# lukifer23/Matrix0

Measured on AMD Instinct MI355X. Metric: self-play games/sec at 800 sims/move, ResNet-24 53M; 1/2/4/8 MI355X, higher is better.
Workload: dtype f16

## Files before the change

matrix0_amd/csrc/attn_block.hip:

```cpp
#include "attn_math.h"
#include "conv_epilogue.h"

typedef float float4v __attribute__((ext_vector_type(4)));

namespace {
constexpr int AB_PIECE = 12288;
constexpr int AB_PIECES_PER_GROUP = 7;
constexpr int AB_GROUPS = 10;
constexpr int AB_X = 0;
constexpr int AB_QK = 81920;
constexpr int AB_VT = AB_QK + 16384;
constexpr int AB_VROW = 68;
constexpr int AB_RING = AB_VT + 4 * 16 * AB_VROW * 2;
constexpr int AB_PAR = AB_RING + 4 * AB_PIECE;
constexpr int AB_LDS = AB_PAR + 4 * 320 * 4;

struct AbLane {
    int tid, lane, w;
    int l15, lq, r31, half;
    int wm, wn;
    size_t b0;
    uint32_t xa[2];
    int wq0, wq1, wpo;
    uint32_t ring_a, of_a;
    const char* wsrc;
    char* ring_w;
    int au, aboard, ahl, aqt, aq;
};
struct AbRegs {
    float4v oc[20];
    float4v qa[2][3];
    half8 fs[2][5];
    half8 of;
    half8 bias8[4];
    half2v visp[16];
};
}

__device__ __forceinline__ void ab_load64(half8& b0, half8& b1, half8& b2, half8& b3, const half8* p) {
    asm volatile("global_load_dwordx4 %0, %4, off\n\tglobal_load_dwordx4 %1, %4, off offset:16\n\t"
                 "global_load_dwordx4 %2, %4, off offset:32\n\tglobal_load_dwordx4 %3, %4, off offset:48"
                 : "=&v"(b0), "=&v"(b1), "=&v"(b2), "=&v"(b3) : "v"(p) : "memory");
}
template <int OFF>
__device__ __forceinline__ void ab_lds16(half8& d, uint32_t addr) {
    asm volatile("ds_read_b128 %0, %1 offset:%2" : "=v"(d) : "v"(addr), "n"(OFF) : "memory");
}
template <int N>
__device__ __forceinline__ void ab_lds_arrived(half8& f0, half8& f1, half8& f2, half8& f3, half8& f4, half8& f5) {
    static_assert(N == 0 || N == 5, "");
    if constexpr (N == 0) asm volatile("s_waitcnt lgkmcnt(0)" : "+v"(f0), "+v"(f1), "+v"(f2), "+v"(f3), "+v"(f4), "+v"(f5) :: "memory");
    else asm volatile("s_waitcnt lgkmcnt(5)" : "+v"(f0), "+v"(f1), "+v"(f2), "+v"(f3), "+v"(f4), "+v"(f5) :: "memory");
}
template <int CTRL>
__device__ __forceinline__ float ab_dpp(float v) {
    return __builtin_bit_cast(float, __builtin_amdgcn_update_dpp(0, __builtin_bit_cast(int, v), CTRL, 0xF, 0xF, true));
}
__device__ __forceinline__ float ab_row_sum(float v) {
    v += ab_dpp<0xB1>(v);
    v += ab_dpp<0x4E>(v);
    v += ab_dpp<0x141>(v);
    v += ab_dpp<0x140>(v);
    return v;
}

#define AB_WAIT(n) asm volatile("s_waitcnt vmcnt(" #n ")" ::: "memory")
#define AB_LGKM0() asm volatile("s_waitcnt lgkmcnt(0)" ::: "memory")

__device__ __forceinline__ char* ab_smem() {
    extern __shared__ __attribute__((aligned(16))) char smem[];
    return smem;
}

__device__ __forceinline__ AbLane ab_lane(const AttnBlockArgs& a) {
    AbLane L;
    L.tid = threadIdx.x; L.lane = L.tid & 63;
    L.w = __builtin_amdgcn_readfirstlane(L.tid >> 6);
    L.l15 = L.lane & 15; L.lq = L.lane >> 4; L.r31 = L.lane & 31; L.half = L.lane >> 5;
    L.wm = L.w >> 1; L.wn = L.w & 1;
    L.b0 = (size_t)blockIdx.x * 2;
    const int l15 = L.l15, lq = L.lq, w = L.w;
    const int xrow0 = 32 * L.wm + l15;
    const int xsw = (xrow0 >> 1) & 7;
    const int xe0 = ((lq ^ xsw) & 7) * 16, xe1 = (((4 + lq) ^ xsw) & 7) * 16;
    const uint32_t lds0 = (uint32_t)(uintptr_t)ab_smem();
    L.xa[0] = lds0 + AB_X + xrow0 * 640 + xe0; L.xa[1] = lds0 + AB_X + xrow0 * 640 + xe1;
    const int wsw = (l15 >> 1) & 7;
    L.wq0 = (3 * L.wn * 16 + l15) * 128 + ((lq ^ wsw) & 7) * 16;
    L.wq1 = (3 * L.wn * 16 + l15) * 128 + (((4 + lq) ^ wsw) & 7) * 16;
    L.wpo = l15 * 64 + ((lq ^ (4 - (l15 >> 2))) & 3) * 16;
    L.ring_a = lds0 + AB_RING;
    L.of_a = lds0 + AB_QK + (lq >> 1) * 4096 + (16 * w + l15) * 32 + ((lq & 1) ^ (l15 >> 3)) * 16;
    L.wsrc = reinterpret_cast<const char*>(a.wpack) + w * 1536 + L.lane * 16;
    L.ring_w = ab_smem() + AB_RING + w * 1536;
    L.au = w >> 1; L.aboard = L.au >> 1; L.ahl = L.au & 1; L.aqt = w & 1;
    L.aq = L.aqt * 32 + L.r31;
    return L;
}

__device__ __forceinline__ void ab_issue(const AbLane& L, int t) {
    const char* s = L.wsrc + (size_t)t * AB_PIECE;
    char* d = L.ring_w + (t & 3) * AB_PIECE;
    glds16(s, d);
    if (L.lane < 32) glds16(s + 1024, d + 1024);
}

__device__ __forceinline__ void ab_prologue(const AttnBlockArgs& a, const AbLane& L) {
    const char* xg = reinterpret_cast<const char*>(a.x) + L.b0 * 64 * 640;
#pragma unroll
    for (int n = 0; n < 10; ++n) {
        const int idx = L.w * 10 + n;
        const int q = idx * 64 + L.lane;
        const int row = q / 40, pos = q - row * 40;
        const int src = (pos & ~7) | ((pos ^ (row >> 1)) & 7);
        glds16(xg + row * 640 + src * 16, ab_smem() + AB_X + idx * 1024);
    }
    ab_issue(L, 0); ab_issue(L, 1); ab_issue(L, 2);
    const int tid = L.tid;
    if (tid < 320) {
        float* par = reinterpret_cast<float*>(ab_smem() + AB_PAR);
        par[tid] = a.ln_g[tid]; par[320 + tid] = a.ln_b[tid];
        par[640 + tid] = a.y2 ? a.gn2_gamma[tid] : 0.f; par[960 + tid] = a.y2 ? a.gn2_beta[tid] : 0.f;
    }
}

__device__ __forceinline__ void ab_visibility(const AttnBlockArgs& a, const AbLane& L, half2v (&visp)[16]) {
    const uint64_t m = a.mask[L.aq];
    static_for<0, 32>([&](auto i_) __attribute__((always_inline)) {
        constexpr int i = decltype(i_)::value;
        constexpr int kt = i >> 4, r = i & 15;
        const int key = kt * 32 + 8 * (r >> 2) + 4 * L.half + (r & 3);
        visp[i >> 1][i & 1] = (_Float16)(float)((m >> key) & 1);
    });
}

__device__ __forceinline__ void ab_zero_qa(float4v (&qa)[2][3]) {
    const float4v zero4 = {0.f, 0.f, 0.f, 0.f};
    static_for<0, 2>([&](auto i_) __attribute__((always_inline)) {
        static_for<0, 3>([&](auto j_) __attribute__((always_inline)) { qa[decltype(i_)::value][decltype(j_)::value] = zero4; });
    });
}

template <bool HP, int U>
__device__ __forceinline__ void ab_load(const AbLane& L, AbRegs& R, const int T) {
    constexpr int S = U & 1, i = U >> 1, kk = U & 1;
    const uint32_t slot = L.ring_a + (uint32_t)(((T + i) & 3) * AB_PIECE);
    if constexpr (HP && i < 2) {
        if constexpr (U == 0) ab_lds16<0>(R.of, L.of_a);
        const uint32_t pa = slot + L.wpo;
        static_for<0, 5>([&](auto jj_) __attribute__((always_inline)) {
            constexpr int jj = decltype(jj_)::value;
            ab_lds16<(5 * kk + jj) * 1024>(R.fs[S][jj], pa);
        });
    } else {
        constexpr int p = i - (HP ? 2 : 0);
        ab_lds16<128 * p>(R.fs[S][3], L.xa[kk]);
        ab_lds16<128 * p + 16 * 640>(R.fs[S][4], L.xa[kk]);
        const uint32_t wa = slot + (kk ? L.wq1 : L.wq0);
        static_for<0, 3>([&](auto j_) __attribute__((always_inline)) {
            constexpr int j = decltype(j_)::value;
            ab_lds16<j * 2048>(R.fs[S][j], wa);
        });
    }
}
template <int U, int N>
__device__ __forceinline__ void ab_arrived(AbRegs& R) {
    constexpr int S = U & 1;
    ab_lds_arrived<N>(R.fs[S][0], R.fs[S][1], R.fs[S][2], R.fs[S][3], R.fs[S][4], R.of);
}
template <bool HP, int U>
__device__ __forceinline__ void ab_mma(AbRegs& R) {
    constexpr int S = U & 1, i = U >> 1, kk = U & 1;
    if constexpr (HP && i < 2) {
        static_for<0, 5>([&](auto jj_) __attribute__((always_inline)) {
            constexpr int c = 10 * i + 5 * kk + decltype(jj_)::value;
            R.oc[c] = __builtin_amdgcn_mfma_f32_16x16x32_f16(R.fs[S][decltype(jj_)::value], R.of, R.oc[c], 0, 0, 0);
        });
    } else {
        static_for<0, 3>([&](auto j_) __attribute__((always_inline)) {
            constexpr int j = decltype(j_)::value;
            R.qa[0][j] = __builtin_amdgcn_mfma_f32_16x16x32_f16(R.fs[S][j], R.fs[S][3], R.qa[0][j], 0, 0, 0);
            R.qa[1][j] = __builtin_amdgcn_mfma_f32_16x16x32_f16(R.fs[S][j], R.fs[S][4], R.qa[1][j], 0, 0, 0);
        });
    }
}

template <bool HP, bool HQ>
__device__ __forceinline__ void ab_sequence(const AttnBlockArgs& a, const AbLane& L, AbRegs& R, const int T, const int g) {
    constexpr int NP = (HP ? 2 : 0) + (HQ ? 5 : 0), NU = 2 * NP;
    constexpr int BU = NU - 3;
    AB_LGKM0();
    AB_WAIT(4);
    __builtin_amdgcn_s_barrier();
    asm volatile("" ::: "memory");
    ab_load<HP, 0>(L, R, T);
    ab_issue(L, T + 3);
    static_for<0, NU>([&](auto u_) __attribute__((always_inline)) {
        constexpr int u = decltype(u_)::value;
        if constexpr (u + 1 < NU) {
            if constexpr (u & 1) {
                ab_arrived<u, 0>(R);
                AB_WAIT(4);
                __builtin_amdgcn_s_barrier();
                asm volatile("" ::: "memory");
            }
            ab_load<HP, u + 1>(L, R, T);
// ... 40 lines not shown
    });
    AB_LGKM0();
    __builtin_amdgcn_s_barrier();
    asm volatile("" ::: "memory");
}

__device__ __forceinline__ void ab_attend(const AbLane& L, AbRegs& R, float isd, float clampv, float wm, float wu) {
    const int half = L.half, r31 = L.r31;
    const char* Kb = ab_smem() + AB_QK + 8192 + L.ahl * 4096 + L.aboard * 64 * 32;
    const int hsw = 16 * (half ^ ((r31 >> 3) & 1));
    const half8 kf0 = *reinterpret_cast<const half8*>(Kb + r31 * 32 + hsw);
    const half8 kf1 = *reinterpret_cast<const half8*>(Kb + (32 + r31) * 32 + hsw);
    char* Qp = ab_smem() + AB_QK + L.ahl * 4096 + (L.aboard * 64 + L.aq) * 32 + hsw;
    const half8 qfr = *reinterpret_cast<const half8*>(Qp);
    half8 vf[2][2];
    attn_v_frags(reinterpret_cast<const _Float16*>(ab_smem() + AB_VT) + (L.au * 16 + L.l15) * AB_VROW, half, vf);
    float16v st[2];
    attn_scores(kf0, kf1, qfr, st);
    asm volatile("s_waitcnt vmcnt(0)" : "+v"(R.bias8[0]), "+v"(R.bias8[1]), "+v"(R.bias8[2]), "+v"(R.bias8[3]) :: "memory");
    auto bias = [&](auto kt_, auto g_) __attribute__((always_inline)) {
        constexpr int bi = decltype(kt_)::value * 16 + 4 * decltype(g_)::value;
        const half8 b = R.bias8[bi >> 3];
        return half4v{b[bi & 7], b[(bi & 7) + 1], b[(bi & 7) + 2], b[(bi & 7) + 3]};
    };
    auto vis = [&](auto kt_, auto g_) __attribute__((always_inline)) {
        constexpr int bi = decltype(kt_)::value * 16 + 4 * decltype(g_)::value;
        return half4v{R.visp[bi >> 1][0], R.visp[bi >> 1][1], R.visp[(bi >> 1) + 1][0], R.visp[(bi >> 1) + 1][1]};
    };
    const uint4v ov = attn_pack_o(attn_softmax_pv(st, bias, vis, vf, isd, clampv, wm, wu), half);
    asm volatile("ds_write_b128 %0, %1" :: "v"((uint32_t)(uintptr_t)Qp), "v"(ov) : "memory");
}

__device__ __forceinline__ half4v* ab_own4(const AbLane& L, int j) {
    const int token = 16 * L.w + L.l15;
    const int chunk = 2 * j + (L.lq >> 1);
    const int tsw = (token >> 1) & 7;
    const int pos = (chunk & ~7) | ((chunk ^ tsw) & 7);
    return reinterpret_cast<half4v*>(ab_smem() + AB_X + token * 640 + (L.lq & 1) * 8 + pos * 16);
}
__device__ __forceinline__ float2* ab_gn_partials() { return reinterpret_cast<float2*>(ab_smem() + AB_RING); }
__device__ __forceinline__ float2* ab_gn_totals() { return ab_gn_partials() + 8 * 20 * 4; }

__device__ __forceinline__ void ab_residual_layernorm(const AttnBlockArgs& a, const AbLane& L, float4v (&oc)[20]) {
    float s1 = 0.f, s2 = 0.f;
    static_for<0, 20>([&](auto j_) __attribute__((always_inline)) {
        constexpr int j = decltype(j_)::value;
        const half4v xv = *ab_own4(L, j);
        static_for<0, 4>([&](auto r_) __attribute__((always_inline)) {
            constexpr int r = decltype(r_)::value;
            const float v = oc[j][r] + (float)xv[r];
            oc[j][r] = v;
            s1 += v; s2 += v * v;
        });
    });
    s1 += __shfl_xor(s1, 16); s2 += __shfl_xor(s2, 16);
    s1 += __shfl_xor(s1, 32); s2 += __shfl_xor(s2, 32);
    const float cnt = (float)a.ln_count;
    const float mean = s1 / cnt;
    float var = s2 / cnt - mean * mean;
    var = var > 0.f ? var : 0.f;
    const float rstd = rsqrtf(var + 1e-5f);
    const float* par = reinterpret_cast<const float*>(ab_smem() + AB_PAR);
    float2* scr = ab_gn_partials();
    const float nmr = -mean * rstd;
    static_for<0, 20>([&](auto j_) __attribute__((always_inline)) {
        constexpr int j = decltype(j_)::value;
        const float4 gm = *reinterpret_cast<const float4*>(par + 16 * j + 4 * L.lq);
        const float4 bt = *reinterpret_cast<const float4*>(par + 320 + 16 * j + 4 * L.lq);
        const float gmv[4] = {gm.x, gm.y, gm.z, gm.w}, btv[4] = {bt.x, bt.y, bt.z, bt.w};
        float p1 = 0.f, p2 = 0.f;
        half4v h;
        static_for<0, 4>([&](auto r_) __attribute__((always_inline)) {
            constexpr int r = decltype(r_)::value;
            const float y = fmaf(fmaf(oc[j][r], rstd, nmr), gmv[r], btv[r]);
            p1 += y; p2 += y * y;
            h[r] = (_Float16)y;
        });
        *ab_own4(L, j) = h;
        p1 = ab_row_sum(p1); p2 = ab_row_sum(p2);
        if (L.l15 == 0) scr[(L.w * 20 + j) * 4 + L.lq] = make_float2(p1, p2);
    });
}

__device__ __forceinline__ void ab_flush(const AbLane& L, _Float16* outp) {
    char* og = reinterpret_cast<char*>(outp) + (L.b0 * 64 + 16 * L.w) * 640;
#pragma unroll
    for (int n = 0; n < 10; ++n) {
        const int q = n * 64 + L.lane;
        const int rl = q / 40, pos = q - rl * 40;
        const int grow = 16 * L.w + rl;
        const int src = (pos & ~7) | ((pos ^ (grow >> 1)) & 7);
        const uint4 v = *reinterpret_cast<const uint4*>(ab_smem() + AB_X + grow * 640 + pos * 16);
        *reinterpret_cast<uint4*>(og + rl * 640 + src * 16) = v;
    }
}

template <int ACT>
__device__ __forceinline__ void ab_second_output(const AbLane& L) {
    const int tid = L.tid;
    float2* scr = ab_gn_partials();
    float2* tot = ab_gn_totals();
    __syncthreads();
    if (tid < 40) {
        const int bd = tid / 20, j = tid - bd * 20;
        float s = 0.f, ss = 0.f;
        for (int ww = 0; ww < 4; ++ww)
            for (int q = 0; q < 4; ++q) { const float2 v = scr[((bd * 4 + ww) * 20 + j) * 4 + q]; s += v.x; ss += v.y; }
        float mu, rstd;
        gn16_mean_rstd(s, ss, mu, rstd);
        tot[tid] = make_float2(mu, rstd);
    }
    __syncthreads();
    float* par = reinterpret_cast<float*>(ab_smem() + AB_PAR);
    {
        float scv[2] = {0.f, 0.f}, shv[2] = {0.f, 0.f};
        if (tid < 320) {
            const float g2 = par[640 + tid], b2 = par[960 + tid];
#pragma unroll
            for (int bd = 0; bd < 2; ++bd) {
                const float2 mr = tot[bd * 20 + (tid >> 4)];
                scv[bd] = g2 * mr.y; shv[bd] = b2 - mr.x * scv[bd];
            }
        }
        __syncthreads();
        if (tid < 320) { par[tid] = scv[0]; par[320 + tid] = shv[0]; par[640 + tid] = scv[1]; par[960 + tid] = shv[1]; }
        __syncthreads();
    }
    static_for<0, 20>([&](auto j_) __attribute__((always_inline)) {
        constexpr int j = decltype(j_)::value;
        const float4 gm = *reinterpret_cast<const float4*>(par + (L.w >> 2) * 640 + 16 * j + 4 * L.lq);
        const float4 bt = *reinterpret_cast<const float4*>(par + (L.w >> 2) * 640 + 320 + 16 * j + 4 * L.lq);
        const float gmv[4] = {gm.x, gm.y, gm.z, gm.w}, btv[4] = {bt.x, bt.y, bt.z, bt.w};
        half4v h = *ab_own4(L, j);
        static_for<0, 4>([&](auto r_) __attribute__((always_inline)) {
            constexpr int r = decltype(r_)::value;
            h[r] = (_Float16)act_fast<ACT>((float)h[r] * gmv[r] + btv[r]);
        });
        *ab_own4(L, j) = h;
    });
}

template <int ACT>
__global__ __launch_bounds__(512) void attn_block_kernel(AttnBlockArgs a) {
    const AbLane L = ab_lane(a);
    ab_prologue(a, L);
    AbRegs R;
    ab_visibility(a, L, R.visp);
    float wm, wu;
    attn_branch_weights(a.mix, wm, wu);
    const float isd = a.inv_sqrt_d * kLog2e;
    const float clampv = 50.f * kLog2e;
    const float4v zero4 = {0.f, 0.f, 0.f, 0.f};
    static_for<0, 20>([&](auto j_) __attribute__((always_inline)) { R.oc[decltype(j_)::value] = zero4; });

    ab_zero_qa(R.qa);
    ab_sequence<false, true>(a, L, R, 0, 0);
#pragma unroll 1
    for (int g = 0; g < AB_GROUPS - 1; ++g) {
        ab_stage_qkv(L, R.qa);
        ab_attend(L, R, isd, clampv, wm, wu);
        ab_zero_qa(R.qa);
        ab_sequence<true, true>(a, L, R, 7 * g + 5, g + 1);
    }
    ab_stage_qkv(L, R.qa);
    ab_attend(L, R, isd, clampv, wm, wu);
    ab_sequence<true, false>(a, L, R, 7 * AB_GROUPS - 2, AB_GROUPS);
    AB_WAIT(0);
    __syncthreads();

    ab_residual_layernorm(a, L, R.oc);
    ab_flush(L, a.y);
    if (a.y2 == nullptr) return;
    ab_second_output<ACT>(L);
    ab_flush(L, a.y2);
}

hipError_t launch_attn_block(const AttnBlockArgs& a, hipStream_t st) {
    if (a.B <= 0 || a.B % 2 != 0 || a.ln_count <= 0 || a.ln_count > 320) return hipErrorInvalidValue;
    if (a.y2 != nullptr && a.act != ACT_SILU && a.act != ACT_RELU) return hipErrorInvalidValue;
    static DeviceOnce once;
    hipError_t e = once.run([] {
        hipError_t r = hipFuncSetAttribute(reinterpret_cast<const void*>(&attn_block_kernel<ACT_SILU>),
                                           hipFuncAttributeMaxDynamicSharedMemorySize, AB_LDS);
        if (r != hipSuccess) return r;
        return hipFuncSetAttribute(reinterpret_cast<const void*>(&attn_block_kernel<ACT_RELU>),
                                   hipFuncAttributeMaxDynamicSharedMemorySize, AB_LDS);
    });
    if (e != hipSuccess) return e;
    const dim3 grid((unsigned)(a.B / 2));
    if (a.act == ACT_RELU) hipLaunchKernelGGL(attn_block_kernel<ACT_RELU>, grid, dim3(512), AB_LDS, st, a);
    else hipLaunchKernelGGL(attn_block_kernel<ACT_SILU>, grid, dim3(512), AB_LDS, st, a);
    return hipGetLastError();
}

size_t attn_block_pack_bytes() { return (size_t)(AB_GROUPS * AB_PIECES_PER_GROUP + 3) * AB_PIECE; }
```

matrix0_amd/csrc/net.h:

```cpp
#pragma once
#include <hip/hip_runtime.h>
#include <stdint.h>
#include <map>
#include <string>
#include <vector>
#include "../../include/m0_engine.h"
#include "net_kernels.h"

struct HostTensor {
    std::vector<float> data;
    std::vector<int64_t> shape;
};

struct PackedGemm {
    _Float16* w = nullptr;
    float* bias = nullptr;
    int taps = 1, Cin = 0, N = 0;
    bool pp = false;
};

struct NormParams {
    float* gamma = nullptr;
    float* beta = nullptr;
};

struct ResBlockW {
    PackedGemm conv1, conv2;
    NormParams bn1, bn2;
    float *se_w1 = nullptr, *se_b1 = nullptr, *se_w2 = nullptr, *se_b2 = nullptr;
    void* se_wf = nullptr;
    int se_hidden = 0;
};

struct AttnW {
    PackedGemm qkv, proj;
    NormParams ln;
    float* rel_bias = nullptr;
    void* blk_w = nullptr;
    _Float16* blk_bias = nullptr;
};

struct TowerLayer {
    int kind;
    int index;
    bool skip;
    int next_bn1 = -1;
};

struct SslHeadW {
    PackedGemm c0, c1;
    NormParams n;
    int out_ch = 0;
};

struct ConvNormOpts {
    const float* posenc = nullptr;
    const _Float16* res = nullptr;
    const NormParams* next_bn1 = nullptr;
};

class Net {
public:
    explicit Net(const m0_net_cfg& cfg, int device, hipStream_t stream);
    ~Net();
    Net* shared_view(hipStream_t stream) const;
    static const char* check_supported(const m0_net_cfg& cfg);
    int load(const char* name, const void* data, int dtype, const int64_t* shape, int ndim, std::string& err);
    int finalize(std::string& err);
    bool ready() const { return finalized_; }
    const std::vector<void*>& device_buffers() const { return dev_allocs_; }
    const std::vector<size_t>& device_buffer_bytes() const { return dev_sizes_; }

    int forward(const float* planes_dev, const _Float16* nhwc_dev, int B, float* logits_dev, float* value_dev,
                float* ssl_dev, hipStream_t st, std::string& err);
    int ensure_workspace(int B, std::string& err);
    int ssl_channels_total() const;
    const m0_net_cfg& cfg() const { return cfg_; }
    size_t param_count() const { return nparams_; }
    double flops_per_position(bool with_ssl) const;
    _Float16* input_nhwc() { return X0_; }
    void set_profile(bool on) { profile_ = on; }
    void harvest_profile();
    double prof_conv_ms() const { return prof_ms_; }
    double prof_conv_flop() const { return prof_flop_; }
    long prof_conv_launches() const { return prof_launches_; }
    void reset_profile() { prof_ms_ = 0; prof_flop_ = 0; prof_launches_ = 0; prof_tail_ms_ = 0; prof_tail_launches_ = 0; }
    double prof_tail_ms() const { return prof_tail_ms_; }
    long prof_tail_launches() const { return prof_tail_launches_; }

private:
    m0_net_cfg cfg_;
    int device_;
    hipStream_t stream_ = nullptr;
    struct Switches { bool fuse_tail = true, fuse_attn = true; } sw_;
    struct Plan {
        bool fuse_tail = false;
        bool fuse_attn = false;
        bool gn_small = false;
        int act = 0, vact = 0;
        int first_bn1 = -1;
    } plan_;
    bool finalized_ = false;
    size_t nparams_ = 0;
    std::map<std::string, HostTensor> sd_;
    std::vector<void*> dev_allocs_;
    std::vector<size_t> dev_sizes_;
    std::vector<void*> ws_allocs_;

    int C_ = 0, Cs_ = 0 ;
    int Cp_ = 0;
    PackedGemm stem_;
    NormParams stem_n_;
    float* posenc_ = nullptr;
    PackedGemm pst_, inter_;
    NormParams pst_n_, inter_n_;
    std::vector<ResBlockW> res_;
    std::vector<AttnW> att_;
    std::vector<TowerLayer> tower_;
    PackedGemm ph_conv_, pfc1_, pfc2_;
    PackedGemm hv_;
    NormParams hv_n_;
    NormParams ph_n_;
    float logit_scale_ = 1.f;
    PackedGemm vh0_, vh3_, vfc1_, vfc2_, vgate_, vfc3_;
    NormParams vh1_n_, vh4_n_;
    std::vector<SslHeadW> ssl_;
    uint64_t* mask_dev_ = nullptr;

    bool profile_ = false;
    std::vector<hipEvent_t> pev_;
    std::vector<double> pflop_;
    std::vector<char> ptail_;
    size_t pev_used_ = 0;
    double prof_ms_ = 0, prof_flop_ = 0, prof_tail_ms_ = 0;
    long prof_launches_ = 0, prof_tail_launches_ = 0;

    int wsB_ = 0, wsM_ = 0;
    _Float16 *X0_ = nullptr, *XA_ = nullptr, *XB_ = nullptr, *T1_ = nullptr, *T2_ = nullptr, *QKV_ = nullptr,
             *O_ = nullptr, *AA_ = nullptr;
    float *S1_ = nullptr, *S2_ = nullptr, *G_ = nullptr;
    _Float16 *PH_ = nullptr, *PH2_ = nullptr, *VH_ = nullptr, *VH2_ = nullptr, *F1_ = nullptr, *F2_ = nullptr,
             *F3_ = nullptr, *F4_ = nullptr, *SH_ = nullptr, *SH2_ = nullptr, *SO_ = nullptr;
    float* VAL_ = nullptr;
    float* SPK_ = nullptr;

    const HostTensor* get(const std::string& k, std::string& err);
    int pack_gemm(PackedGemm& g, const std::string& wkey, const std::string& bkey, int taps, int Cin_real,
                  int Cin_pad, int N_real, int N_pad, int k_perm_ch, std::string& err, int qkv_heads = 0,
                  int qkv_heads_pad = 0);
    int pack_attn_block(AttnW& a, const std::string& prefix, std::string& err);
    int pack_chess_features(std::string& err);
    int pack_se(ResBlockW& r, const std::string& prefix, std::string& err);
    int pack_attn(AttnW& a, bool skip, const std::string& prefix, std::string& err);
    void upload_attn_mask();
    int pack_joint_head(std::string& err);
    int pack_ssl_heads(std::string& err);
    void make_plan();
    int upload_norm(NormParams& n, const std::string& prefix, int C_real, int C_pad, std::string& err);
    float* upload_f32(const std::vector<float>& v);
    void* dalloc(size_t bytes, bool ws);
    const NormParams* bn1(int res_index) const { return res_index < 0 ? nullptr : &res_[res_index].bn1; }
    template <class Launch>
    hipError_t profiled(bool on, hipStream_t st, double flop, bool tail, Launch&& launch);
    hipError_t run_gemm(const PackedGemm& g, GemmArgs a, hipStream_t st);
    hipError_t conv_norm_act(const PackedGemm& g, const NormParams& n, const _Float16* in, _Float16* out, _Float16* scratch,
                             int Mrows, hipStream_t st, const ConvNormOpts& o = ConvNormOpts());
    hipError_t se_gate(const ResBlockW& r, const float* stats, int boards, hipStream_t st);
};
```

matrix0_amd/csrc/net.hip:

```cpp
#include "net.h"
#include "attn_math.h"
#include <math.h>
#include <string.h>
#include <algorithm>
#include <stdlib.h>

static inline int ceil_to(int v, int m) { return (v + m - 1) / m * m; }

static const char* kSslNames[5] = {"piece", "threat", "pin", "fork", "control"};
static const int kSslOut[5] = {13, 1, 1, 1, 3};

const char* Net::check_supported(const m0_net_cfg& c) {
    if (!c.norm_group) return "HIP path supports norm='group' only (BatchNorm configs are not built)";
    if (!c.preact) return "HIP path supports preact=true only";
    if (c.channels % 32 != 0 || c.channels < 32 || c.channels > 384) return "channels must be a multiple of 32 in [32,384]";
    if (c.planes < 1 || c.planes > 32) return "planes must be in [1,32]";
    if (c.attention && (c.attention_heads <= 0 || c.channels % c.attention_heads != 0 ||
                        c.channels / c.attention_heads != 16))
        return "attention head_dim (channels/attention_heads) must be 16";
    if (c.activation != M0_ACT_SILU && c.activation != M0_ACT_RELU) return "activation must be silu or relu";
    if (c.blocks < 1) return "blocks must be >= 1";
    if (c.policy_factor_rank < 0) return "policy_factor_rank must be >= 0";
    if (c.self_supervised && c.ssl_tasks && (c.channels / 2) % 16 != 0) return "ssl heads need channels/2 % 16 == 0";
    return nullptr;
}

Net::Net(const m0_net_cfg& cfg, int device, hipStream_t stream) : cfg_(cfg), device_(device), stream_(stream) {
    auto off = [](const char* name) { const char* e = getenv(name); return e && e[0] == '0'; };
    sw_.fuse_tail = !off("M0_FUSE_TAIL");
    sw_.fuse_attn = !off("M0_FUSE_ATTN");
    C_ = cfg.channels;
    Cp_ = (C_ > 256 && C_ < 320) ? 320 : C_;
    Cs_ = ceil_to(std::max(16, C_ / 2), 32);
    int k = cfg.attention_every_k;
    int stride = std::max(1, cfg.infer_attention_stride);
    int att_seen = 0;
    for (int i = 0; i < cfg.blocks; ++i) {
        tower_.push_back({0, (int)res_.size(), false});
        res_.emplace_back();
        if (cfg.attention && k > 0 && (i % k) == (k - 1)) {
            ++att_seen;
            bool skip = stride > 1 && (att_seen % stride) != 0;
            tower_.push_back({1, (int)att_.size(), skip});
            att_.emplace_back();
        }
    }
}

Net* Net::shared_view(hipStream_t stream) const {
    Net* v = new Net(*this);
    v->stream_ = stream;
    v->dev_allocs_.clear(); v->dev_sizes_.clear();
    v->ws_allocs_.clear(); v->wsB_ = 0; v->wsM_ = 0;
    v->sd_.clear();
    v->pev_.clear(); v->pflop_.clear(); v->ptail_.clear(); v->pev_used_ = 0; v->profile_ = false;
    v->prof_ms_ = v->prof_flop_ = v->prof_tail_ms_ = 0; v->prof_launches_ = v->prof_tail_launches_ = 0;
    return v;
}

Net::~Net() {
    for (hipEvent_t e : pev_) (void)hipEventDestroy(e);
    for (void* p : dev_allocs_) (void)hipFree(p);
    for (void* p : ws_allocs_) (void)hipFree(p);
}

void* Net::dalloc(size_t bytes, bool ws) {
    void* p = nullptr;
    if (bytes == 0) bytes = 16;
    if (hipMalloc(&p, bytes) != hipSuccess) return nullptr;
    (void)hipMemsetAsync(p, 0, bytes, stream_);
    if (!ws) (void)hipStreamSynchronize(stream_);
    (ws ? ws_allocs_ : dev_allocs_).push_back(p);
    if (!ws) dev_sizes_.push_back(bytes);
    return p;
}

float* Net::upload_f32(const std::vector<float>& v) {
    float* d = (float*)dalloc(v.size() * 4, false);
    if (d && !v.empty()) (void)hipMemcpy(d, v.data(), v.size() * 4, hipMemcpyHostToDevice);
    return d;
}

int Net::load(const char* name, const void* data, int dtype, const int64_t* shape, int ndim, std::string& err) {
    if (finalized_) { err = "weights already finalized"; return M0_ERR_STATE; }
    if (!name || (!data && ndim >= 0)) { err = "null argument"; return M0_ERR_INVALID; }
    HostTensor t;
    size_t n = 1;
    for (int i = 0; i < ndim; ++i) { t.shape.push_back(shape[i]); n *= (size_t)shape[i]; }
    t.data.resize(n);
    if (dtype == 0) memcpy(t.data.data(), data, n * 4);
    else if (dtype == 1) {
        const _Float16* h = (const _Float16*)data;
        for (size_t i = 0; i < n; ++i) t.data[i] = (float)h[i];
    } else { err = "dtype must be 0 (f32) or 1 (f16)"; return M0_ERR_INVALID; }
    std::string key(name);
    if (cfg_.policy_factor_rank > 0 && key.rfind("policy_fc.", 0) == 0) key = "policy_fc1." + key.substr(10);
    sd_[key] = std::move(t);
    return M0_OK;
}

const HostTensor* Net::get(const std::string& k, std::string& err) {
    auto it = sd_.find(k);
    if (it == sd_.end()) { err = "missing state-dict key: " + k; return nullptr; }
    return &it->second;
}

int Net::pack_gemm(PackedGemm& g, const std::string& wkey, const std::string& bkey, int taps, int Cin_real,
                   int Cin_pad, int N_real, int N_pad, int k_perm_ch, std::string& err, int qkv_heads, int qkv_heads_pad) {
    const HostTensor* w = get(wkey, err);
    if (!w) return M0_ERR_INVALID;
    size_t expect = (size_t)N_real * Cin_real * taps;
    if (w->data.size() != expect) { err = "shape mismatch for " + wkey; return M0_ERR_INVALID; }
    nparams_ += expect;
// ... 489 lines not shown
        }
    }
    pev_used_ = 0;
    pflop_.clear();
    ptail_.clear();
}

#define KCHK(x)                                                                           \
    do {                                                                                  \
        hipError_t e_ = (x);                                                              \
        if (e_ != hipSuccess) {                                                           \
            err = std::string("kernel launch failed: ") + #x + ": " + hipGetErrorString(e_); \
            return M0_ERR_HIP;                                                            \
        }                                                                                 \
    } while (0)

int Net::forward(const float* planes_dev, const _Float16* nhwc_dev, int B, float* logits_dev, float* value_dev,
                 float* ssl_dev, hipStream_t st, std::string& err) {
    if (!finalized_) { err = "weights not finalized"; return M0_ERR_STATE; }
    if (B <= 0) { err = "batch must be positive"; return M0_ERR_INVALID; }
    TRY(ensure_workspace(B, err));
    const int Bp = ceil_to(B, 4);
    const int Mc = Bp * 64;
    const int Mfc = ceil_to(B, 256);
    const int act = plan_.act, vact = plan_.vact;
    const int C = Cp_;

    const _Float16* x0 = nhwc_dev;
    if (!x0) {
        if (!planes_dev) { err = "no input"; return M0_ERR_INVALID; }
        KCHK(launch_planes_to_nhwc(planes_dev, X0_, B, cfg_.planes, st));
        x0 = X0_;
    }
    _Float16* xa = XA_;
    _Float16* xb = XB_;
    const NormParams* first_bn1 = bn1(plan_.first_bn1);
    ConvNormOpts so;
    if (cfg_.chess_features) so.posenc = posenc_; else so.next_bn1 = first_bn1;
    KCHK(conv_norm_act(stem_, stem_n_, x0, xa, T1_, Mc, st, so));
    if (cfg_.chess_features) {
        if (cfg_.piece_square_tables) {
            ConvNormOpts po;
            po.res = xa;
            KCHK(conv_norm_act(pst_, pst_n_, xa, xb, T1_, Mc, st, po));
            std::swap(xa, xb);
        }
        ConvNormOpts io;
        io.res = xa; io.next_bn1 = first_bn1;
        KCHK(conv_norm_act(inter_, inter_n_, xa, xb, T1_, Mc, st, io));
        std::swap(xa, xb);
    }
    for (const TowerLayer& L : tower_) {
        const NormParams* next_bn1 = bn1(L.next_bn1);
        if (L.kind == 0) {
            const ResBlockW& r = res_[L.index];
            KCHK(conv_norm_act(r.conv1, r.bn2, AA_, T1_, T2_, Mc, st));
            if (plan_.fuse_tail) {
                GemmArgs a = gemm_args(r.conv2, T1_, xb, Mc, act);
                a.res = xa;
                if (next_bn1) { a.y2 = AA_; a.gn_gamma = next_bn1->gamma; a.gn_beta = next_bn1->beta; }
                if (cfg_.se) { a.se_w1 = r.se_w1; a.se_b1 = r.se_b1; a.se_w2 = r.se_w2; a.se_b2 = r.se_b2; a.se_hidden = r.se_hidden;
                               a.se_wf = r.se_wf; }
                KCHK(profiled(profile_, st, conv3x3_flop(r.conv2, Mc), true, [&] { return launch_conv_gemm(a, 9, st); }));
            } else {
                GemmArgs a = gemm_args(r.conv2, T1_, T2_, Mc);
                a.out_stats = S2_;
                KCHK(run_gemm(r.conv2, a, st));
                EwArgs e = ew_args(T2_, xb, C, act);
                e.t_stats = S2_; e.res = xa;
                if (cfg_.se) { KCHK(se_gate(r, S2_, Bp, st)); e.gate = G_; }
                ew_next_bn1(e, next_bn1, AA_);
                KCHK(launch_ew_board(e, Bp, st));
            }
        } else {
            if (L.skip) continue;
            const AttnW& w = att_[L.index];
            const float inv_sqrt_d = 1.f / sqrtf((float)(C_ / cfg_.attention_heads));
            if (plan_.fuse_attn && w.blk_w != nullptr) {
                AttnBlockArgs ab;
                memset(&ab, 0, sizeof(ab));
                ab.x = xa; ab.wpack = w.blk_w; ab.bias = w.blk_bias; ab.mask = mask_dev_;
                ab.ln_g = w.ln.gamma; ab.ln_b = w.ln.beta; ab.y = xb;
                if (next_bn1) { ab.y2 = AA_; ab.gn2_gamma = next_bn1->gamma; ab.gn2_beta = next_bn1->beta; }
                ab.B = Bp; ab.ln_count = C_; ab.act = act; ab.mix = cfg_.attention_unmasked_mix; ab.inv_sqrt_d = inv_sqrt_d;
                KCHK(launch_attn_block(ab, st));
            } else {
                KCHK(run_gemm(w.qkv, gemm_args(w.qkv, xa, QKV_, Mc), st));
                AttnArgs aa;
                aa.qkv = QKV_; aa.rel_bias = w.rel_bias; aa.mask = mask_dev_; aa.o = O_;
                aa.B = Bp; aa.H = C / 16; aa.C = C; aa.mix = cfg_.attention_unmasked_mix;
                aa.inv_sqrt_d = inv_sqrt_d;
                KCHK(launch_attn_core(aa, st));
                KCHK(run_gemm(w.proj, gemm_args(w.proj, O_, T1_, Mc), st));
                EwArgs e = ew_args(T1_, xb, C, act);
                e.res = xa; e.ln_g = w.ln.gamma; e.ln_b = w.ln.beta; e.ln_count = C_;
                ew_next_bn1(e, next_bn1, AA_);
                KCHK(launch_ew_board(e, Bp, st));
            }
        }
        std::swap(xa, xb);
    }
    const bool joint = plan_.gn_small;
    if (joint) {
        GemmArgs a = gemm_args(hv_, xa, PH2_, Mc, act);
        a.gn_gamma = hv_n_.gamma; a.gn_beta = hv_n_.beta;
        a.ldo = 64; a.out2 = VH2_; a.ldo2 = 128; a.nsplit = 64;
        KCHK(launch_conv_gemm(a, 1, st));
    } else {
        KCHK(conv_norm_act(ph_conv_, ph_n_, xa, PH2_, PH_, Mc, st));
    }
    const bool factored = cfg_.policy_factor_rank > 0;
    if (factored) KCHK(run_gemm(pfc1_, gemm_args(pfc1_, PH2_, F1_, Mfc, ACT_RELU), st));
    const PackedGemm& plast = factored ? pfc2_ : pfc1_;
    GemmArgs pl = gemm_args(plast, factored ? F1_ : PH2_, logits_dev, Mfc);
    pl.Mvalid = B; pl.out_f32 = 1; pl.out_scale = logit_scale_;
    KCHK(run_gemm(plast, pl, st));
    if (!joint) KCHK(conv_norm_act(vh0_, vh1_n_, xa, VH2_, VH_, Mc, st));
    _Float16* vflat = joint ? VH_ : VH2_;
    KCHK(conv_norm_act(vh3_, vh4_n_, VH2_, vflat, VH_, Mc, st));
    KCHK(run_gemm(vfc1_, gemm_args(vfc1_, vflat, F2_, Mfc, vact), st));
    KCHK(run_gemm(vfc2_, gemm_args(vfc2_, F2_, F3_, Mfc, vact), st));
    GemmArgs vg = gemm_args(vgate_, F3_, F4_, Mfc, ACT_SIGMOID);
    vg.mul = F3_;
    KCHK(run_gemm(vgate_, vg, st));
    GemmArgs v3 = gemm_args(vfc3_, F4_, VAL_, Mfc, ACT_TANH);
    v3.out_f32 = 1;
    KCHK(run_gemm(vfc3_, v3, st));
    KCHK(hipMemcpy2DAsync(value_dev, 4, VAL_, 32 * 4, 4, B, hipMemcpyDeviceToDevice, st));
    if (ssl_dev && !ssl_.empty()) {
        const int ctot = ssl_channels_total();
        int coff = 0;
        for (auto& h : ssl_) {
            KCHK(conv_norm_act(h.c0, h.n, xa, SH2_, SH_, Mc, st));
            KCHK(run_gemm(h.c1, gemm_args(h.c1, SH2_, SO_, Mc), st));
            KCHK(launch_nhwc_to_nchw_f32(SO_, ssl_dev, B, 32, h.out_ch, ctot, coff, st));
            coff += h.out_ch;
        }
    }
    return M0_OK;
}
```

matrix0_amd/csrc/net_kernels.h:

```cpp
#pragma once
#include <hip/hip_runtime.h>
#include <stdint.h>

enum { ACT_NONE = 0, ACT_RELU = 1, ACT_SILU = 2, ACT_LEAKY = 3, ACT_SIGMOID = 4, ACT_TANH = 5 };

enum ConvEpi {
    EPI_PLAIN,
    EPI_GN,
    EPI_ELEMENT,
    EPI_TAIL,
    EPI_TAIL_PRE,
};

constexpr int TAIL_SE_HMAX = 96;

struct GemmArgs {
    const _Float16* in;
    const _Float16* w;
    void* out;
    const float* gn_gamma;
    const float* gn_beta;
    const float* bias;
    const _Float16* mul;
    float* out_stats;
    int Mrows;
    int Mvalid;
    int Cin;
    int N;
    int Npad;
    int ldo;
    int epi_act;
    int out_f32;
    float out_scale;
    int ksplit;
    int w_pp;
    const _Float16* res;
    const float* pre_gamma;
    const float* pre_beta;
    _Float16* y2;
    const float* se_w1;
    const float* se_b1;
    const float* se_w2;
    const float* se_b2;
    int se_hidden;
    const void* se_wf;
    const float* posenc;
    void* out2;
    int ldo2;
    int nsplit;
};

struct EwArgs {
    const _Float16* t;
    const float* t_stats;
    const float* gn_gamma;
    const float* gn_beta;
    const float* gate;
    const _Float16* res;
    const float* posenc;
    const float* ln_g;
    const float* ln_b;
    int ln_count;
    _Float16* y;
    float* out_stats;
    _Float16* y2;
    const float* gn2_gamma;
    const float* gn2_beta;
    int C;
    int act;
};

struct SeGateArgs {
    const float* t_stats;
    const float* w1;
    const float* b1;
    const float* w2;
    const float* b2;
    float* gate;
    int B, C, hidden, act;
};

struct AttnArgs {
    const _Float16* qkv;
    const float* rel_bias;
    const uint64_t* mask;
    _Float16* o;
    int B, H, C;
    float mix;
    float inv_sqrt_d;
};

struct AttnBlockArgs {
    const _Float16* x;
    const void* wpack;
    const _Float16* bias;
    const uint64_t* mask;
    const float* ln_g;
    const float* ln_b;
    const float* gn2_gamma;
    const float* gn2_beta;
    _Float16* y;
    _Float16* y2;
    int B;
    int ln_count;
    int act;
    float mix;
    float inv_sqrt_d;
};
hipError_t launch_attn_block(const AttnBlockArgs& a, hipStream_t st);
hipError_t launch_splitk_reduce(const float* part, int splits, int M, int N, const float* bias, int act, _Float16* out,
                                hipStream_t st);
size_t attn_block_pack_bytes();

hipError_t launch_conv_gemm(const GemmArgs& a, int taps, hipStream_t st);
int conv_gemm_tile_n(int Cin, int Npad);
int conv_gemm_kc(int Cin, int Npad);
hipError_t launch_ew_board(const EwArgs& a, int boards, hipStream_t st);
hipError_t launch_se_gate(const SeGateArgs& a, hipStream_t st);
hipError_t launch_attn_core(const AttnArgs& a, hipStream_t st);
hipError_t launch_planes_to_nhwc(const float* x, void* y, int B, int P, hipStream_t st);
hipError_t launch_nhwc_to_nchw_f32(const void* x, float* y, int B, int ld, int n, int ctot, int coff, hipStream_t st);
```

Before: 1.165.

## Make fused attention block persistent and prefetch next board pair during flush

New measurement: 1.179, median of 6. 1.2% higher.

```diff
diff --git a/matrix0_amd/csrc/attn_block.hip b/matrix0_amd/csrc/attn_block.hip
--- a/matrix0_amd/csrc/attn_block.hip
+++ b/matrix0_amd/csrc/attn_block.hip
@@ -19,7 +19,6 @@
     int tid, lane, w;
     int l15, lq, r31, half;
     int wm, wn;
-    size_t b0;
     uint32_t xa[2];
     int wq0, wq1, wpo;
     uint32_t ring_a, of_a;
@@ -35,12 +34,30 @@
     half8 bias8[4];
     half2v visp[16];
 };
+struct AbNext {
+    half8 x[10];
+    float par[4];
+};
 }
 
 __device__ __forceinline__ void ab_load64(half8& b0, half8& b1, half8& b2, half8& b3, const half8* p) {
     asm volatile("global_load_dwordx4 %0, %4, off\n\tglobal_load_dwordx4 %1, %4, off offset:16\n\t"
                  "global_load_dwordx4 %2, %4, off offset:32\n\tglobal_load_dwordx4 %3, %4, off offset:48"
                  : "=&v"(b0), "=&v"(b1), "=&v"(b2), "=&v"(b3) : "v"(p) : "memory");
+}
+__device__ __forceinline__ void ab_gload16(half8& d, int off, const void* base) {
+    asm volatile("global_load_dwordx4 %0, %1, %2" : "+v"(d) : "v"(off), "s"(base) : "memory");
+}
+__device__ __forceinline__ void ab_gload4(float& d, int off, const void* base) {
+    asm volatile("global_load_dword %0, %1, %2" : "+v"(d) : "v"(off), "s"(base) : "memory");
+}
+template <int OFF>
+__device__ __forceinline__ void ab_lds_store16(uint32_t addr, const half8& v) {
+    asm volatile("ds_write_b128 %0, %1 offset:%2" :: "v"(addr), "v"(v), "n"(OFF) : "memory");
+}
+template <int OFF>
+__device__ __forceinline__ void ab_lds_store4(uint32_t addr, float v) {
+    asm volatile("ds_write_b32 %0, %1 offset:%2" :: "v"(addr), "v"(v), "n"(OFF) : "memory");
 }
 template <int OFF>
 __device__ __forceinline__ void ab_lds16(half8& d, uint32_t addr) {
@@ -78,7 +95,6 @@
     L.w = __builtin_amdgcn_readfirstlane(L.tid >> 6);
     L.l15 = L.lane & 15; L.lq = L.lane >> 4; L.r31 = L.lane & 31; L.half = L.lane >> 5;
     L.wm = L.w >> 1; L.wn = L.w & 1;
-    L.b0 = (size_t)blockIdx.x * 2;
     const int l15 = L.l15, lq = L.lq, w = L.w;
     const int xrow0 = 32 * L.wm + l15;
     const int xsw = (xrow0 >> 1) & 7;
@@ -98,23 +114,33 @@
     return L;
 }
 
+__device__ __forceinline__ void ab_per_pass(AbLane& L) {
+    asm volatile("" : "+v"(L.lane), "+v"(L.l15), "+v"(L.lq), "+v"(L.r31), "+v"(L.half), "+v"(L.aq), "+v"(L.xa[0]), "+v"(L.xa[1]),
+                      "+v"(L.wq0), "+v"(L.wq1), "+v"(L.wpo), "+v"(L.of_a), "+v"(L.wsrc));
+}
 __device__ __forceinline__ void ab_issue(const AbLane& L, int t) {
     const char* s = L.wsrc + (size_t)t * AB_PIECE;
     char* d = L.ring_w + (t & 3) * AB_PIECE;
     glds16(s, d);
-    if (L.lane < 32) glds16(s + 1024, d + 1024);
-}
-
-__device__ __forceinline__ void ab_prologue(const AttnBlockArgs& a, const AbLane& L) {
-    const char* xg = reinterpret_cast<const char*>(a.x) + L.b0 * 64 * 640;
+    int lane = L.lane;
+    asm volatile("" : "+v"(lane));
+    if (lane < 32) glds16(s + 1024, d + 1024);
+}
+
+__device__ __forceinline__ int ab_x_source(const AbLane& L, int n) {
+    const int q = (L.w * 10 + n) * 64 + L.lane;
+    const int row = q / 40, pos = q - row * 40;
+    const int src = (pos & ~7) | ((pos ^ (row >> 1)) & 7);
+    return row * 640 + src * 16;
+}
+__device__ __forceinline__ const char* ab_pair_rows(const AttnBlockArgs& a, int pair) {
+    return reinterpret_cast<const char*>(a.x) + (size_t)pair * (128 * 640);
+}
+
+__device__ __forceinline__ void ab_prologue(const AttnBlockArgs& a, const AbLane& L, int pair) {
+    const char* xg = ab_pair_rows(a, pair);
 #pragma unroll
-    for (int n = 0; n < 10; ++n) {
-        const int idx = L.w * 10 + n;
-        const int q = idx * 64 + L.lane;
-        const int row = q / 40, pos = q - row * 40;
-        const int src = (pos & ~7) | ((pos ^ (row >> 1)) & 7);
-        glds16(xg + row * 640 + src * 16, ab_smem() + AB_X + idx * 1024);
-    }
+    for (int n = 0; n < 10; ++n) glds16(xg + ab_x_source(L, n), ab_smem() + AB_X + (L.w * 10 + n) * 1024);
     ab_issue(L, 0); ab_issue(L, 1); ab_issue(L, 2);
     const int tid = L.tid;
     if (tid < 320) {
@@ -122,6 +148,44 @@
         par[tid] = a.ln_g[tid]; par[320 + tid] = a.ln_b[tid];
         par[640 + tid] = a.y2 ? a.gn2_gamma[tid] : 0.f; par[960 + tid] = a.y2 ? a.gn2_beta[tid] : 0.f;
     }
+}
+
+__device__ __forceinline__ void ab_define_next(AbNext& N) {
+    asm volatile("" : "=v"(N.x[0]), "=v"(N.x[1]), "=v"(N.x[2]), "=v"(N.x[3]), "=v"(N.x[4]), "=v"(N.x[5]), "=v"(N.x[6]), "=v"(N.x[7]),
+                      "=v"(N.x[8]), "=v"(N.x[9]), "=v"(N.par[0]), "=v"(N.par[1]), "=v"(N.par[2]), "=v"(N.par[3]));
+}
+__device__ __forceinline__ void ab_request_next(const AttnBlockArgs& a, const AbLane& L, int pair, AbNext& N) {
+    const char* xg = ab_pair_rows(a, pair);
+    static_for<0, 10>([&](auto n_) __attribute__((always_inline)) {
+        constexpr int n = decltype(n_)::value;
+        ab_gload16(N.x[n], ab_x_source(L, n), xg);
+    });
+    if (a.y2 != nullptr && L.w < 5) {
+        const int po = L.tid * 4;
+        ab_gload4(N.par[0], po, a.ln_g); ab_gload4(N.par[1], po, a.ln_b);
+        ab_gload4(N.par[2], po, a.gn2_gamma); ab_gload4(N.par[3], po, a.gn2_beta);
+    }
+}
+__device__ __forceinline__ void ab_next_arrived(const AttnBlockArgs& a, const AbLane& L, AbNext& N) {
+    AB_LGKM0();
+    __builtin_amdgcn_s_barrier();
+    asm volatile("s_waitcnt vmcnt(0)"
+                 : "+v"(N.x[0]), "+v"(N.x[1]), "+v"(N.x[2]), "+v"(N.x[3]), "+v"(N.x[4]), "+v"(N.x[5]), "+v"(N.x[6]), "+v"(N.x[7]),
+                   "+v"(N.x[8]), "+v"(N.x[9]), "+v"(N.par[0]), "+v"(N.par[1]), "+v"(N.par[2]), "+v"(N.par[3]) :: "memory");
+    const uint32_t lds0 = (uint32_t)(uintptr_t)ab_smem();
+    const uint32_t xd = lds0 + AB_X + L.w * 10240 + L.lane * 16;
+    static_for<0, 10>([&](auto n_) __attribute__((always_inline)) {
+        constexpr int n = decltype(n_)::value;
+        ab_lds_store16<n * 1024>(xd, N.x[n]);
+    });
+    if (a.y2 != nullptr && L.w < 5) {
+        const uint32_t pd = lds0 + AB_PAR + L.tid * 4;
+        static_for<0, 4>([&](auto i_) __attribute__((always_inline)) {
+            constexpr int i = decltype(i_)::value;
+            ab_lds_store4<i * 1280>(pd, N.par[i]);
+        });
+    }
+    ab_issue(L, 0); ab_issue(L, 1); ab_issue(L, 2);
 }
 
 __device__ __forceinline__ void ab_visibility(const AttnBlockArgs& a, const AbLane& L, half2v (&visp)[16]) {
@@ -328,8 +392,8 @@
     });
 }
 
-__device__ __forceinline__ void ab_flush(const AbLane& L, _Float16* outp) {
-    char* og = reinterpret_cast<char*>(outp) + (L.b0 * 64 + 16 * L.w) * 640;
+__device__ __forceinline__ void ab_flush(const AbLane& L, _Float16* outp, int pair) {
+    char* og = reinterpret_cast<char*>(outp) + ((size_t)pair * 128 + 16 * L.w) * 640;
 #pragma unroll
     for (int n = 0; n < 10; ++n) {
         const int q = n * 64 + L.lane;
@@ -388,8 +452,10 @@
 
 template <int ACT>
 __global__ __launch_bounds__(512) void attn_block_kernel(AttnBlockArgs a) {
-    const AbLane L = ab_lane(a);
-    ab_prologue(a, L);
+    AbLane L = ab_lane(a);
+    const int pairs = a.B >> 1, stride = (int)gridDim.x;
+    int pair = (int)blockIdx.x;
+    ab_prologue(a, L, pair);
     AbRegs R;
     ab_visibility(a, L, R.visp);
     float wm, wu;
@@ -397,43 +463,71 @@
     const float isd = a.inv_sqrt_d * kLog2e;
     const float clampv = 50.f * kLog2e;
     const float4v zero4 = {0.f, 0.f, 0.f, 0.f};
-    static_for<0, 20>([&](auto j_) __attribute__((always_inline)) { R.oc[decltype(j_)::value] = zero4; });
-
-    ab_zero_qa(R.qa);
-    ab_sequence<false, true>(a, L, R, 0, 0);
+
 #pragma unroll 1
-    for (int g = 0; g < AB_GROUPS - 1; ++g) {
+    for (;;) {
+        ab_per_pass(L);
+        static_for<0, 20>([&](auto j_) __attribute__((always_inline)) { R.oc[decltype(j_)::value] = zero4; });
+        ab_zero_qa(R.qa);
+        ab_sequence<false, true>(a, L, R, 0, 0);
+#pragma unroll 1
+        for (int g = 0; g < AB_GROUPS - 1; ++g) {
+            ab_stage_qkv(L, R.qa);
+            ab_attend(L, R, isd, clampv, wm, wu);
+            ab_zero_qa(R.qa);
+            ab_sequence<true, true>(a, L, R, 7 * g + 5, g + 1);
+        }
         ab_stage_qkv(L, R.qa);
         ab_attend(L, R, isd, clampv, wm, wu);
-        ab_zero_qa(R.qa);
-        ab_sequence<true, true>(a, L, R, 7 * g + 5, g + 1);
-    }
-    ab_stage_qkv(L, R.qa);
-    ab_attend(L, R, isd, clampv, wm, wu);
-    ab_sequence<true, false>(a, L, R, 7 * AB_GROUPS - 2, AB_GROUPS);
-    AB_WAIT(0);
-    __syncthreads();
-
-    ab_residual_layernorm(a, L, R.oc);
-    ab_flush(L, a.y);
-    if (a.y2 == nullptr) return;
-    ab_second_output<ACT>(L);
-    ab_flush(L, a.y2);
+        ab_sequence<true, false>(a, L, R, 7 * AB_GROUPS - 2, AB_GROUPS);
+        AB_WAIT(0);
+        __syncthreads();
+
+        ab_residual_layernorm(a, L, R.oc);
+        const int next = pair + stride;
+        const bool more = next < pairs;
+        AbNext N;
+        ab_define_next(N);
+        if (more) ab_request_next(a, L, next, N);
+        ab_flush(L, a.y, pair);
+        if (a.y2 != nullptr) {
+            ab_second_output<ACT>(L);
+            ab_flush(L, a.y2, pair);
+        }
+        if (!more) break;
+        ab_next_arrived(a, L, N);
+        pair = next;
+    }
 }
 
 hipError_t launch_attn_block(const AttnBlockArgs& a, hipStream_t st) {
-    if (a.B <= 0 || a.B % 2 != 0 || a.ln_count <= 0 || a.ln_count > 320) return hipErrorInvalidValue;
+    if (a.B <= 0 || a.B % 2 != 0 || a.ln_count <= 0 || a.ln_count > 320 || a.grid_cap < 0) return hipErrorInvalidValue;
     if (a.y2 != nullptr && a.act != ACT_SILU && a.act != ACT_RELU) return hipErrorInvalidValue;
     static DeviceOnce once;
-    hipError_t e = once.run([] {
+    static std::atomic<int> cu_count[32];
+    int cus = 0;
+    hipError_t e = once.run([&cus] {
         hipError_t r = hipFuncSetAttribute(reinterpret_cast<const void*>(&attn_block_kernel<ACT_SILU>),
                                            hipFuncAttributeMaxDynamicSharedMemorySize, AB_LDS);
         if (r != hipSuccess) return r;
-        return hipFuncSetAttribute(reinterpret_cast<const void*>(&attn_block_kernel<ACT_RELU>),
-                                   hipFuncAttributeMaxDynamicSharedMemorySize, AB_LDS);
+        r = hipFuncSetAttribute(reinterpret_cast<const void*>(&attn_block_kernel<ACT_RELU>),
+                                hipFuncAttributeMaxDynamicSharedMemorySize, AB_LDS);
+        if (r != hipSuccess) return r;
+        int d = 0;
+        if ((r = hipGetDevice(&d)) != hipSuccess) return r;
+        if ((r = hipDeviceGetAttribute(&cus, hipDeviceAttributeMultiprocessorCount, d)) != hipSuccess) return r;
+        if (cus <= 0) return hipErrorInvalidDevice;
+        if ((unsigned)d < 32u) cu_count[d].store(cus, std::memory_order_relaxed);
+        return hipSuccess;
     });
     if (e != hipSuccess) return e;
-    const dim3 grid((unsigned)(a.B / 2));
+    if (cus == 0) {
+        int d = 0;
+        if ((e = hipGetDevice(&d)) != hipSuccess) return e;
+        cus = cu_count[d].load(std::memory_order_relaxed);
+    }
+    const int pairs = a.B / 2, cap = a.grid_cap > 0 ? a.grid_cap : cus;
+    const dim3 grid((unsigned)(pairs < cap ? pairs : cap));
     if (a.act == ACT_RELU) hipLaunchKernelGGL(attn_block_kernel<ACT_RELU>, grid, dim3(512), AB_LDS, st, a);
     else hipLaunchKernelGGL(attn_block_kernel<ACT_SILU>, grid, dim3(512), AB_LDS, st, a);
     return hipGetLastError();
diff --git a/matrix0_amd/csrc/net.h b/matrix0_amd/csrc/net.h
--- a/matrix0_amd/csrc/net.h
+++ b/matrix0_amd/csrc/net.h
@@ -92,7 +92,7 @@
     m0_net_cfg cfg_;
     int device_;
     hipStream_t stream_ = nullptr;
-    struct Switches { bool fuse_tail = true, fuse_attn = true; } sw_;
+    struct Switches { bool fuse_tail = true, fuse_attn = true; int attn_grid = 0; } sw_;
     struct Plan {
         bool fuse_tail = false;
         bool fuse_attn = false;
diff --git a/matrix0_amd/csrc/net.hip b/matrix0_amd/csrc/net.hip
--- a/matrix0_amd/csrc/net.hip
+++ b/matrix0_amd/csrc/net.hip
@@ -29,6 +29,7 @@
     auto off = [](const char* name) { const char* e = getenv(name); return e && e[0] == '0'; };
     sw_.fuse_tail = !off("M0_FUSE_TAIL");
     sw_.fuse_attn = !off("M0_FUSE_ATTN");
+    if (const char* e = getenv("M0_ATTN_GRID")) sw_.attn_grid = std::max(0, atoi(e));
     C_ = cfg.channels;
     Cp_ = (C_ > 256 && C_ < 320) ? 320 : C_;
     Cs_ = ceil_to(std::max(16, C_ / 2), 32);
@@ -684,7 +685,7 @@
                 ab.x = xa; ab.wpack = w.blk_w; ab.bias = w.blk_bias; ab.mask = mask_dev_;
                 ab.ln_g = w.ln.gamma; ab.ln_b = w.ln.beta; ab.y = xb;
                 if (next_bn1) { ab.y2 = AA_; ab.gn2_gamma = next_bn1->gamma; ab.gn2_beta = next_bn1->beta; }
-                ab.B = Bp; ab.ln_count = C_; ab.act = act; ab.mix = cfg_.attention_unmasked_mix; ab.inv_sqrt_d = inv_sqrt_d;
+                ab.B = Bp; ab.ln_count = C_; ab.act = act; ab.grid_cap = sw_.attn_grid; ab.mix = cfg_.attention_unmasked_mix; ab.inv_sqrt_d = inv_sqrt_d;
                 KCHK(launch_attn_block(ab, st));
             } else {
                 KCHK(run_gemm(w.qkv, gemm_args(w.qkv, xa, QKV_, Mc), st));
diff --git a/matrix0_amd/csrc/net_kernels.h b/matrix0_amd/csrc/net_kernels.h
--- a/matrix0_amd/csrc/net_kernels.h
+++ b/matrix0_amd/csrc/net_kernels.h
@@ -104,6 +104,7 @@
     int B;
     int ln_count;
     int act;
+    int grid_cap;
     float mix;
     float inv_sqrt_d;
 };
```
